# toverainc/willow-inference-server

Measured on NVIDIA H100. Metric: Whisper large-v2 realtime multiple (audio s / s), beam 5, 3.84 s utterance, higher is better.
Workload: dtype f16

## Files before the change

willow_inference_server_b200/csrc/decoder.cuh:

```cuda
#pragma once
#include "common.cuh"
#include "kernels.h"

namespace wisb {

constexpr int DEC_MAX_ROWS = 8;
constexpr int MAX_BEAM = 8;
constexpr int MAX_CAND = 2 * MAX_BEAM;
constexpr int TOPK_CHUNKS = 32;

struct DecState {
  int pos;
  int gen_step;
  int n_done;
  int all_done;
  int ticket;
};

enum GemvEpi : int {
  GV_STORE = 0,
  GV_RESID = 1,
  GV_GELU = 2,
  GV_QKV = 3,
};
// ... 16 lines not shown
  int* cand_idx = nullptr;
  int* tokens = nullptr;
  int* seq[2] = {nullptr, nullptr};
  int* indir[2] = {nullptr, nullptr};
  int* flip = nullptr;
  int* done = nullptr;
  int* n_hyp = nullptr;
  float* best_score = nullptr;
  int* best_len = nullptr;
  int* best_tokens = nullptr;
  DecState* st = nullptr;
  int* row_pos = nullptr;
  int* row_slot = nullptr;
  const int* max_new_u = nullptr;
  float rep_penalty = 1.f;
  int no_repeat_ngram = 0;
  const int* beam_u = nullptr;
  const int* max_hyp_u = nullptr;
  const float* lp_u = nullptr;
  int sample = 0;
  int topk = 0;
  float temperature = 1.f;
  const unsigned long long* seed_u = nullptr;
};
void search_step_run(const SearchArgs& a, cudaStream_t stream);
void prefill_advance_run(int* tokens, const int* prompt , int prompt_len, int R, int beam,
                         DecState* st, cudaStream_t stream);
void search_init_run(const SearchArgs& a, const int* prompt, cudaStream_t stream, int shared_prefix = 0);
void prefill_rows_run(int* tokens, int* row_pos, int* row_slot, const int* prompt, int prompt_len, int n_utt, int p0,
                      int chunk, int beam, cudaStream_t stream);

struct BatchLayer {
  GemmPlan qkv, o, cq, co, fc1, fc2;
  const float *ln1g = nullptr, *ln1b = nullptr;
  const float *ob = nullptr, *ln2g = nullptr, *ln2b = nullptr;
  const float *cob = nullptr, *ln3g = nullptr, *ln3b = nullptr;
  const float *fc2b = nullptr, *next_g = nullptr, *next_b = nullptr;
  const __half* ck = nullptr;
  const __half* cv = nullptr;
  __half* kcache = nullptr;
  __half* vcache = nullptr;
};
struct BatchArgs {
  int R = 0, d = 0, H = 0, n_utt = 0, rows_per_utt = 0, t_cap = 0, t_ind = 0, prefill = 0, with_logits = 0, pdl = 0;
  int wide = 0;
  const int* tokens = nullptr;
  const int* row_pos = nullptr;
  const int* row_slot = nullptr;
  const __half* tok_emb = nullptr;
  const float* pos_emb = nullptr;
  float* x = nullptr;
// ... 106 lines not shown
```

willow_inference_server_b200/csrc/engine.cu:

```cuda
#include <stdio.h>
#include <string.h>

#include <algorithm>
#include <cmath>
#include <functional>
#include <map>
#include <memory>
#include <mutex>
#include <string>
#include <vector>

#include "../../include/wisb200.h"
#include "decoder.cuh"
#include "kernels.h"

namespace wisb {

namespace {

thread_local std::string g_last_error;

struct TensorRef {
  const uint8_t* ptr = nullptr;
  int dtype = 0, ndim = 0;
// ... 91 lines not shown
  int mel_B = 0;
  DevBuf<__half> enc_in;
  int enc_in_B = 0;
  int enc_cap = 0;
  DevBuf<__half> h1, xn, qkv, vt, ctx, hbuf, enc_out, ckv;
  DevBuf<float> x;
  GemmPlan plan_conv2, plan_ckv;
  CUtensorMap ckv_map;
  CUtensorMap ckv_map_plain;
  std::vector<EncLayerPlans> enc_plans;
  AttnPlan attn_plan;
  int plans_B = 0, plans_vmn = -1, plans_pdl = -1;
  DevBuf<float> dx, dq, dctx, dh, logits;
  DevBuf<__half> dctx16, dh16, dxn16, dq16;
  DevBuf<float> dxstat;
  DevBuf<__half> kcache, vcache;
  DevBuf<uint8_t> mask_base, mask_cur;
  std::vector<int> mask_extra;
  DevBuf<float> row_lse, cum, cand_score, best_score, lang_probs, part_max, part_sum;
  DevBuf<unsigned long long> part;
  DevBuf<int> cand_idx, tokens, seq0, seq1, ind0, ind1, flip, done, n_hyp, best_len, best_tokens, prompt_dev, lang_ids;
  DevBuf<DecState> st;
  DevBuf<int> row_pos, row_slot, max_new_u;
  DevBuf<int> beam_u, max_hyp_u;
  DevBuf<float> lp_u;
  DevBuf<unsigned long long> seed_u;
  int search_rows = 0;
  int search_gen = 0, bd_search_gen = -1;
  int batch_rows = 320, batch_pdl = 1, decoder_batch = 1, cross_tc = 1, debug_chunk = 1;
  int bd_rows = 0, bd_tcap = 0, bd_launches_step = 0;
  DevBuf<float> bx, bq, bpart, blogits;
  DevBuf<__half> bxn, bctx, bh, bkc, bvc;
  std::vector<BatchLayer> bd_layers;
  GemmPlan bd_vocab;
  int wide_prefill = 1, prefill_rows = 1024;
  int pf_rows = 0, pf_tcap = 0;
  size_t pf_layer_cache = 0;
  const __half* pf_kc = nullptr;
  DevBuf<float> px, pq, ppart;
  DevBuf<__half> pxn, pctx, ph;
  DevBuf<int> ptok, ppos, pslot;
  std::vector<BatchLayer> pf_layers;
  DevBuf<MegaLayer> mega_layers;
  DevBuf<__half> mega_img;
  int enc_pdl = 1;
  int mega_mma = 1;
// ... 260 lines not shown
    WISB_CUDA(cudaMemcpy(h->al_items.p, items.data(), A * 4, cudaMemcpyHostToDevice));
    WISB_CUDA(cudaMemcpy(h->al_head.p, heads.data(), A * 4, cudaMemcpyHostToDevice));
  }
  h->mask_base.ensure(d.n_vocab);
  h->mask_cur.ensure(d.n_vocab);
  WISB_CUDA(cudaMemcpy(h->mask_base.p, mask.data(), mask.size(), cudaMemcpyHostToDevice));
  WISB_CUDA(cudaMemcpy(h->mask_cur.p, mask.data(), mask.size(), cudaMemcpyHostToDevice));
  const size_t R = DEC_MAX_ROWS;
  h->dx.ensure(R * d.d_model, true);
  h->dq.ensure(R * d.d_model, true);
  h->dctx.ensure(R * d.d_model, true);
  h->dh.ensure(R * 4 * d.d_model, true);
  h->dctx16.ensure(R * d.d_model, true);
  h->dh16.ensure(R * 4 * d.d_model, true);
  h->dxn16.ensure(R * d.d_model, true);
  h->dq16.ensure(R * d.d_model, true);
  h->dxstat.ensure(static_cast<size_t>(h->num_sms) * R * 2, true);
  h->logits.ensure(R * d.n_vocab_pad, true);
  const size_t cache = static_cast<size_t>(d.n_dec_layers) * R * T_MAX * d.d_model;
  h->kcache.ensure(cache, true);
  h->vcache.ensure(cache, true);
  h->flip.ensure(1, true);
  h->st.ensure(1, true);
  ensure_search(h, DEC_MAX_ROWS);
  h->mega_layers.ensure(d.n_dec_layers);
  h->mega_layers_host.ensure(d.n_dec_layers);
  h->mega_flags.ensure(mega_flags_words(), true);
  h->cross_flags.ensure(static_cast<size_t>(DEC_MAX_ROWS) * d.n_heads * 16 * 32, true);
  {
    const size_t per_layer = 2ull * (3 * d.d_model + d.d_model + 4 * d.d_model);
    h->ln_fold.ensure(per_layer * d.n_dec_layers + 2ull * d.n_vocab_pad);
    for (int i = 0; i < d.n_dec_layers; ++i) {
      const DecLayerW& w = h->dec_w[i];
      float* base = h->ln_fold.p + per_layer * i;
      mega_ln_fold(w.qkvw, w.ln1g, w.ln1b, w.qkvb, base, base + 3 * d.d_model, 3 * d.d_model, d.d_model, h->stream);
      base += 6 * d.d_model;
      mega_ln_fold(w.cqw, w.ln2g, w.ln2b, w.cqb, base, base + d.d_model, d.d_model, d.d_model, h->stream);
      base += 2 * d.d_model;
      mega_ln_fold(w.fc1w, w.ln3g, w.ln3b, w.fc1b, base, base + 4 * d.d_model, 4 * d.d_model, d.d_model, h->stream);
    }
    float* vb = h->ln_fold.p + per_layer * d.n_dec_layers;
    mega_ln_fold(h->H("dec.tok_emb"), h->F("dec.ln.g"), h->F("dec.ln.b"), nullptr, vb, vb + d.n_vocab_pad, d.n_vocab, d.d_model, h->stream);
  }
  if (mega_k_chunks(4 * d.d_model) > 1) {
    const size_t per = static_cast<size_t>(4) * d.d_model * d.d_model;
    h->fc2_chunked.ensure(per * d.n_dec_layers);
// ... 314 lines not shown
  a.prompt_len = c.prompt_len;
  a.length_penalty = c.lp;
  a.row_lse = h->row_lse.p;
  a.part_max = h->part_max.p;
  a.part_sum = h->part_sum.p;
  a.cum = h->cum.p;
  a.part = h->part.p;
  a.cand_score = h->cand_score.p;
  a.cand_idx = h->cand_idx.p;
  a.tokens = h->tokens.p;
  a.seq[0] = h->seq0.p;
  a.seq[1] = h->seq1.p;
  a.indir[0] = h->ind0.p;
  a.indir[1] = h->ind1.p;
  a.flip = h->flip.p;
  a.done = h->done.p;
  a.n_hyp = h->n_hyp.p;
  a.best_score = h->best_score.p;
  a.best_len = h->best_len.p;
  a.best_tokens = h->best_tokens.p;
  a.st = h->st.p;
  a.row_pos = h->row_pos.p;
  a.row_slot = h->row_slot.p;
  a.max_new_u = c.per_utt_max_new ? h->max_new_u.p : nullptr;
  a.rep_penalty = c.rep_penalty;
  a.no_repeat_ngram = c.no_repeat_ngram;
  if (c.mixed) {
    a.beam_u = h->beam_u.p;
    a.max_hyp_u = h->max_hyp_u.p;
    a.lp_u = h->lp_u.p;
  }
  if (c.sample) {
    a.sample = 1;
    a.topk = c.topk;
    a.temperature = c.temperature;
    a.seed_u = h->seed_u.p;
  }
  if (c.ts) {
    a.ts = 1;
    a.no_ts = dm.no_timestamps;
    a.ts_begin = dm.no_timestamps + 1;
    a.ts_max_init = std::min(a.ts_begin + c.ts_max_init, dm.n_vocab - 1);
  }
  return a;
}

// ... 36 lines not shown
      m.o.shape = m.cq.shape = m.co.shape = 1;
      m.fc1.shape = 2;
      m.fc2.shape = 3;
      m.o.next_g = w.ln2g;
      m.co.next_g = w.ln3g;
      m.fc2.next_g = i + 1 < dm.n_dec_layers ? h->dec_w[i + 1].ln1g : h->F("dec.ln.g");
      const size_t dd = d;
      const __half* img = h->mega_img.p + 14 * dd * dd * i;
      m.qkv.w = img;
      m.o.w = img + 3 * dd * dd;
      m.cq.w = img + 4 * dd * dd;
      m.co.w = img + 5 * dd * dd;
      m.fc1.w = img + 6 * dd * dd;
      m.fc2.w = img + 10 * dd * dd;
    }
    bind_cross_kv(h, m, i, c.u0, c.B_total);
    m.kcache = h->kcache.p + i * layer_cache;
    m.vcache = h->vcache.p + i * layer_cache;
  }
  WISB_CUDA(cudaMemcpyAsync(h->mega_layers.p, h->mega_layers_host.p, sizeof(MegaLayer) * dm.n_dec_layers,
                            cudaMemcpyHostToDevice, h->stream));
}

void enqueue_decoder_forward(wisb_handle* h, const DecodeCfg& c, bool with_logits, bool prefill_pass = false) {
  const Dims& dm = h->dims;
  MegaArgs a;
  a.layers = h->mega_layers.p;
  a.n_layers = dm.n_dec_layers;
  a.vocab.w = h->H("dec.tok_emb");
  a.vocab.ln_g = h->F("dec.ln.g");
  {
    const size_t per_layer = 2ull * 8 * dm.d_model;
    const float* vb = h->ln_fold.p + per_layer * dm.n_dec_layers;
    a.vocab.ln_s2 = vb;
    a.vocab.bias = vb + dm.n_vocab_pad;
  }
  a.vocab.x = h->dx.p;
  a.vocab.out = h->logits.p;
  a.vocab.ldo = dm.n_vocab_pad;
  a.vocab.N = dm.n_vocab;
  a.vocab.K = dm.d_model;
  a.vocab.epi = GV_STORE;
  if (h->mega_mma) {
    a.vocab.w = h->mega_img.p + static_cast<size_t>(14) * dm.d_model * dm.d_model * dm.n_dec_layers;
    a.tc = 1;
    a.ctx16 = h->dctx16.p;
    a.xn16 = h->dxn16.p;
    a.q16 = h->dq16.p;
    a.xstat = h->dxstat.p;
    a.vocab.x16 = h->dxn16.p;
    a.vocab.shape = 4;
  }
  a.with_logits = with_logits ? 1 : 0;
  a.R = c.n_utt * c.beam;
  a.d = dm.d_model;
  a.H = dm.n_heads;
  a.n_utt = c.n_utt;
  a.beam = c.beam;
  a.t_max = T_MAX;
  a.tokens = h->tokens.p;
  if (prefill_pass) {
    a.pf_len = c.prompt_len - 1;
    a.pf_tok_stride = c.prompt_len;
    a.pf_slot_stride = c.beam;
    a.R = c.n_utt * a.pf_len;
    a.beam = a.pf_len;
    a.tokens = h->prompt_dev.p;
  }
  a.tok_emb = h->H("dec.tok_emb");
  a.pos_emb = h->F("dec.pos");
  a.x = h->dx.p;
  a.q = h->dq.p;
  a.ctx = h->dctx.p;
  a.indir0 = h->ind0.p;
  a.indir1 = h->ind1.p;
  a.flip = h->flip.p;
  a.st = h->st.p;
  a.cross_part = h->cross_part.p;
  a.cross_flags = h->cross_flags.p;
  a.epoch_base = h->mega_flags.p;
  dec_pass_run(a, h->num_sms, h->stream);
}

void enqueue_prefill(wisb_handle* h, const DecodeCfg& c) {
  enqueue_decoder_forward(h, c, false);
// ... 72 lines not shown
        out_len[o] = len;
        for (int t = 0; t < len && t < out_stride; ++t) out_ids[o * out_stride + t] = toks[static_cast<size_t>(r) * mn + t];
        if (out_score) out_score[o] = cap > 0 ? sc[k] : 0.f;
      }
    }
    return;
  }
  int* lens = h->pin_i.p + 4;
  int* toks = lens + c.n_utt;
  const int mn = c.max_new > 0 ? c.max_new : 1;
  WISB_CUDA(cudaMemcpyAsync(lens, h->best_len.p, sizeof(int) * c.n_utt, cudaMemcpyDeviceToHost, s));
  WISB_CUDA(cudaMemcpyAsync(toks, h->best_tokens.p, sizeof(int) * c.n_utt * mn, cudaMemcpyDeviceToHost, s));
  WISB_CUDA(cudaMemcpyAsync(h->pin_f.p, h->best_score.p, sizeof(float) * c.n_utt, cudaMemcpyDeviceToHost, s));
  WISB_CUDA(cudaStreamSynchronize(s));
  for (int u = 0; u < c.n_utt; ++u) {
    const int cap = c.per_utt_max_new ? max_new_host[c.u0 + u] : c.max_new;
    const int len = cap > 0 ? lens[u] : 0;
    out_len[c.u0 + u] = len;
    for (int t = 0; t < len && t < out_stride; ++t) out_ids[static_cast<size_t>(c.u0 + u) * out_stride + t] = toks[u * mn + t];
    if (out_score) out_score[c.u0 + u] = cap > 0 ? h->pin_f.p[u] : 0.f;
  }
}

void persistent_setup(wisb_handle* h, const DecodeCfg& c, const int32_t* prompts, const int* max_new_host,
                      int shared_prefix = 0) {
  upload_prompts(h, prompts, max_new_host, c);
  search_init_run(make_search_args(h, c), h->prompt_dev.p, h->stream, shared_prefix);
  upload_mega_layers(h, c);
}

int step_loop(wisb_handle* h, int max_new, bool look_ahead, const std::function<int()>& enqueue) {
  cudaStream_t s = h->stream;
  volatile int* flag = h->pin_i.p;
  flag[0] = flag[1] = 0;
  if (look_ahead && h->ev_flag[0] == nullptr) {
    WISB_CUDA(cudaEventCreateWithFlags(&h->ev_flag[0], cudaEventDisableTiming));
    WISB_CUDA(cudaEventCreateWithFlags(&h->ev_flag[1], cudaEventDisableTiming));
  }
  int steps = 0;
  for (int gs = 0; gs < max_new; ++gs) {
    h->launches += enqueue();
    ++steps;
    WISB_CUDA(cudaMemcpyAsync(const_cast<int*>(flag) + (gs & 1), &h->st.p->all_done, sizeof(int), cudaMemcpyDeviceToHost, s));
    if (!look_ahead) {
      WISB_CUDA(cudaStreamSynchronize(s));
      if (flag[gs & 1]) break;
      continue;
    }
    WISB_CUDA(cudaEventRecord(h->ev_flag[gs & 1], s));
    if (gs >= 1) {
      WISB_CUDA(cudaEventSynchronize(h->ev_flag[(gs - 1) & 1]));
      if (flag[(gs - 1) & 1]) {
        --steps;
        break;
      }
    }
  }
  return steps;
}

int wide_prefill_run(wisb_handle* h, const DecodeCfg& c, int chunk, __half* kc, __half* vc, size_t layer_cache, int t_cap);

int decode_pass(wisb_handle* h, const DecodeCfg& c, const int32_t* prompts, const int* max_new_host, int32_t* out_ids,
                int out_stride, int32_t* out_len, float* out_score) {
  int steps = 0;
  const int pf_rows = c.n_utt * (c.prompt_len - 1);
  const bool one_pass_prefill = c.prompt_len > 1 && pf_rows <= DEC_MAX_ROWS && c.prompt_len - 1 <= MAX_BEAM;
  const bool wide = h->wide_prefill && c.prompt_len - 1 > MAX_BEAM;
  persistent_setup(h, c, prompts, max_new_host, one_pass_prefill || wide ? 1 : 0);
  if (c.max_new > 0) {
    if (one_pass_prefill) {
      enqueue_decoder_forward(h, c, false, true);
      ++steps;
    } else if (wide) {
      const int chunk = std::min(c.prompt_len - 1, std::max(1, h->prefill_rows / c.n_utt));
      steps += wide_prefill_run(h, c, chunk, h->kcache.p, h->vcache.p, static_cast<size_t>(DEC_MAX_ROWS) * T_MAX * h->dims.d_model,
                                T_MAX);
    } else {
      for (int p = 0; p + 1 < c.prompt_len; ++p) {
        enqueue_prefill(h, c);
        ++steps;
      }
    }
    if (!wide) h->launches += (c.prompt_len - 1) * 2;
    steps += step_loop(h, c.max_new, true, [&] {
      enqueue_step(h, c);
      return 1 + 2;
    });
  }
  read_results(h, c, max_new_host, out_ids, out_stride, out_len, out_score);
  return steps;
}


void plan_dec_gemm(wisb_handle* h, GemmPlan& p, const __half* a, long long lda, const __half* w, int M, int N, int K,
                   GemmEpi e, bool allow_split) {
  const int mt = M / 128;
  int bn = 256;
  while (bn > 64 && (N % bn != 0 || mt * (N / bn) < 120)) bn /= 2;
  int splits = 1;
  if (allow_split) {
    const int kb = K / 64;
    while (mt * (N / bn) * splits < 120 && splits < 8 && kb % (splits * 2) == 0 && kb / (splits * 2) >= 4) splits *= 2;
    e.mode = EPI_F32;
    e.split_stride = static_cast<long long>(M) * N;
  }
  gemm_plan(p, a, lda, w, M, N, K, e, h->num_sms, bn, 0, splits);
}

void plan_batch_layers(wisb_handle* h, std::vector<BatchLayer>& layers, int Rp, float* q, __half* xn, __half* ctx,
                       __half* hid, float* part, __half* kc, __half* vc, size_t layer_cache, int t_cap, const int* row_slot,
// ... 31 lines not shown
    GemmEpi eq;
    eq.mode = EPI_F32;
    eq.bias = w.cqb;
    eq.out = q;
    eq.ldo = d;
    plan_dec_gemm(h, b.cq, xn, d, w.cqw, Rp, d, d, eq, false);
    plan_dec_gemm(h, b.co, ctx, d, w.cow, Rp, d, d, ep, true);
    GemmEpi e1;
    e1.mode = EPI_F16_GELU;
    e1.bias = w.fc1b;
    e1.out = hid;
    e1.ldo = 4 * d;
    plan_dec_gemm(h, b.fc1, xn, d, w.fc1w, Rp, 4 * d, d, e1, false);
    plan_dec_gemm(h, b.fc2, hid, 4LL * d, w.fc2w, Rp, d, 4 * d, ep, true);
  }
}

void ensure_batch(wisb_handle* h, int rows, int t_need) {
  const Dims& dm = h->dims;
  const int d = dm.d_model, L = dm.n_dec_layers;
  int Rp = round_up(rows, 128);
  int tc = round_up(t_need, 32);
  if (tc > T_MAX) tc = T_MAX;
  ensure_search(h, rows);
  if (Rp <= h->bd_rows && tc <= h->bd_tcap && h->bd_search_gen == h->search_gen) return;
  if (Rp < h->bd_rows) Rp = h->bd_rows;
  if (tc < h->bd_tcap) tc = h->bd_tcap;
  WISB_CUDA(cudaStreamSynchronize(h->stream));
  drop_graphs(h);
  const size_t M = static_cast<size_t>(Rp);
  h->bx.ensure(M * d, true);
  h->bq.ensure(M * d, true);
  h->bxn.ensure(M * d, true);
  h->bctx.ensure(M * d, true);
  h->bh.ensure(M * 4 * d, true);
  h->bpart.ensure(8 * M * d, true);
  h->blogits.ensure(M * dm.n_vocab_pad, true);
  const size_t layer_cache = M * tc * d;
  if (layer_cache * L > h->bkc.n) {
    h->bkc.release();
    h->bvc.release();
  }
  h->bkc.ensure(layer_cache * L, true);
  h->bvc.ensure(layer_cache * L, true);
  plan_batch_layers(h, h->bd_layers, Rp, h->bq.p, h->bxn.p, h->bctx.p, h->bh.p, h->bpart.p, h->bkc.p, h->bvc.p,
                    layer_cache, tc, h->row_slot.p, h->row_pos.p);
  {
// ... 140 lines not shown
    a.xn = h->pxn.p;
    a.q = h->pq.p;
    a.ctx = h->pctx.p;
    a.part = h->ppart.p;
    a.part_stride = static_cast<long long>(h->pf_rows) * h->dims.d_model;
    if (h->ckv_is_sw) a.ckv_map = &h->ckv_map_plain;
    h->launches += 1 + batch_pass_run(a, h->pf_layers.data(), L, h->stream);
  }
  return passes;
}

void bind_batch_cross_kv(wisb_handle* h, int u0, int B_total) {
  for (int i = 0; i < h->dims.n_dec_layers; ++i) bind_cross_kv(h, h->bd_layers[i], i, u0, B_total);
}

int decode_batch(wisb_handle* h, const DecodeCfg& c, const int32_t* prompts, const int* max_new_host, int32_t* out_ids,
                 int out_stride, int32_t* out_len, float* out_score) {
  cudaStream_t s = h->stream;
  ensure_batch(h, c.n_utt * c.beam, c.prompt_len + c.max_new);
  bind_batch_cross_kv(h, c.u0, c.B_total);
  int steps = 0;
  upload_prompts(h, prompts, max_new_host, c);
  if (c.max_new > 0) {
    const int chunk_max = std::max(1, std::min(h->bd_rows / c.n_utt, MAX_BEAM));
    const int wide = std::min(c.prompt_len - 1, std::max(chunk_max, h->prefill_rows / c.n_utt));
    if (h->wide_prefill && c.prompt_len - 1 > MAX_BEAM && wide > chunk_max)
      steps += wide_prefill_run(h, c, wide, h->bkc.p, h->bvc.p, static_cast<size_t>(h->bd_rows) * h->bd_tcap * h->dims.d_model,
                                h->bd_tcap);
    else
      steps += batch_prefill(h, c, c.prompt_len, c.prompt_len - 1, chunk_max, c.beam, false);
    search_init_run(make_batch_search_args(h, c), h->prompt_dev.p, s, 1);
    cudaGraphExec_t g = nullptr;
    if (h->use_graphs && !h->profile) {
      GraphKey key;
      memset(&key, 0, sizeof(key));
      key.n_utt = c.n_utt; key.beam = c.beam; key.prompt_len = c.prompt_len; key.max_new = c.max_new;
      key.max_hyp = c.mixed ? 0 : c.max_hyp; key.lp = c.mixed ? 0.f : c.lp; key.u0 = c.u0; key.b_total = c.B_total;
      key.mixed = c.mixed;
      key.per_utt_max_new = c.per_utt_max_new;
      key.ts = c.ts; key.ts_max_init = c.ts ? c.ts_max_init : 0;
      key.rep_penalty = c.rep_penalty; key.no_repeat_ngram = c.no_repeat_ngram;
      key.sample = c.sample; key.topk = c.sample ? c.topk : 0; key.temperature = c.sample ? c.temperature : 0.f;
      auto it = h->graphs.find(key);
      if (it == h->graphs.end()) {
        if (h->graphs.size() > 64) drop_graphs(h);
        cudaGraph_t graph;
        cudaGraphExec_t exec;
        WISB_CUDA(cudaStreamBeginCapture(s, cudaStreamCaptureModeThreadLocal));
        enqueue_batch_step(h, c);
        WISB_CUDA(cudaStreamEndCapture(s, &graph));
        WISB_CUDA(cudaGraphInstantiate(&exec, graph, 0));
        WISB_CUDA(cudaGraphDestroy(graph));
        it = h->graphs.emplace(key, exec).first;
      }
      g = it->second;
    }
    steps += step_loop(h, c.max_new, false, [&] {
      if (g) WISB_CUDA(cudaGraphLaunch(g, s)); else enqueue_batch_step(h, c);
      return h->bd_launches_step;
    });
  }
  read_results(h, c, max_new_host, out_ids, out_stride, out_len, out_score);
  return steps;
}

constexpr size_t ALIGN_WS_BYTES = 2ull << 30;

void align_group(wisb_handle* h, int g0, int n, const int32_t* start_seq, int S, const int32_t* text, const int32_t* text_len,
                 int text_stride, const int32_t* num_frames, int width, int n_max, int f_max, int32_t* out_path,
                 int path_stride, int32_t* out_path_len, float* out_token_probs, float* cap_out) {
  const Dims& dm = h->dims;
  cudaStream_t s = h->stream;
  const int A = h->al_A;
  int n_grp = 0;
  for (int u = 0; u < n; ++u) n_grp = std::max(n_grp, static_cast<int>(text_len[g0 + u]));
  const int total = S + 1 + n_grp;
  int P = round_up(total, MAX_BEAM);
  if (P > dm.n_text_ctx) P = dm.n_text_ctx;
  ensure_batch(h, n * MAX_BEAM, P);
  bind_batch_cross_kv(h, 0, n);
  const int ts = std::max(text_stride, 1);
  std::vector<int> tok(static_cast<size_t>(n) * P, dm.eot), nt(n), nf(n), txt(static_cast<size_t>(n) * ts, 0);
  for (int u = 0; u < n; ++u) {
// ... 927 lines not shown
    a.row_pos = d_i.p + o_rpos;
    a.row_slot = d_slot.p;
    a.done = d_i.p + o_done;
    a.n_hyp = d_i.p + o_nhyp;
    a.best_len = d_i.p + o_blen;
    a.best_tokens = d_i.p + o_btok;
    a.cum = d_f.p;
    a.best_score = d_f.p + R;
    a.max_new_u = max_new_u ? d_cap.p : nullptr;
    a.rep_penalty = rep_penalty;
    a.no_repeat_ngram = no_repeat_ngram;
    if (mixed) {
      a.beam_u = d_beam.p;
      a.max_hyp_u = d_hyp.p;
      a.lp_u = d_lp.p;
    }
    if (sample) {
      a.sample = 1;
      a.topk = topk;
      a.temperature = temperature;
      a.seed_u = d_seed.p;
    }
    static_assert(sizeof(DecState) == 5 * sizeof(int), "DecState is five ints");
    if (init) search_init_run(a, d_prompt.p, s, init - 1);
    search_step_run(a, s);
    WISB_CUDA(cudaMemcpyAsync(state_i, d_i.p, sizeof(int) * n_i, cudaMemcpyDeviceToHost, s));
    WISB_CUDA(cudaMemcpyAsync(state_f, d_f.p, sizeof(float) * n_f, cudaMemcpyDeviceToHost, s));
    WISB_CUDA(cudaMemcpyAsync(cand_idx, d_ci.p, sizeof(int) * n_utt * MAX_CAND, cudaMemcpyDeviceToHost, s));
    WISB_CUDA(cudaMemcpyAsync(cand_score, d_cs.p, sizeof(float) * n_utt * MAX_CAND, cudaMemcpyDeviceToHost, s));
    WISB_CUDA(cudaMemcpyAsync(row_lse, d_lse.p, sizeof(float) * R, cudaMemcpyDeviceToHost, s));
    WISB_CUDA(cudaStreamSynchronize(s));
  });
}

static void align_impl(wisb_handle* h, const float* mel, int B, const int32_t* start_seq, int start_len, const int32_t* text,
                       const int32_t* text_len, int text_stride, const int32_t* num_frames, int median_filter_width,
                       int32_t* out_path, int path_stride, int32_t* out_path_len, float* out_token_probs, float* cap_out) {
    const Dims& dm = h->dims;
    WISB_REQUIRE(h->blob != nullptr, "handle has no model (created by wisb_create_frontend)");
    WISB_REQUIRE(B >= 1 && B <= 4096, "B out of range");
    WISB_REQUIRE(start_seq != nullptr && text_len != nullptr && num_frames != nullptr && out_path != nullptr &&
                 out_path_len != nullptr && out_token_probs != nullptr, "NULL argument");
    WISB_REQUIRE(start_len >= 1 && start_seq[0] == dm.sot, "start_sequence must begin with <|startoftranscript|>");
    for (int i = 0; i < start_len; ++i)
      WISB_REQUIRE(start_seq[i] >= 0 && start_seq[i] < dm.no_timestamps,
                   "start_sequence must not contain <|notimestamps|> or timestamp tokens");
    WISB_REQUIRE(median_filter_width >= 1 && median_filter_width <= 31 && median_filter_width % 2 == 1,
// ... 496 lines not shown
    DecodeCfg c;
    c.u0 = 0; c.n_utt = n_utt; c.B_total = n_utt; c.beam = beam; c.prompt_len = pf_len + 1; c.max_new = 1; c.max_hyp = 1; c.lp = 1.f;
    const DecState st{pf_len > 0 ? 0 : pos, 0, 0, 0, 0};
    WISB_CUDA(cudaMemcpyAsync(h->st.p, &st, sizeof(DecState), cudaMemcpyHostToDevice, s));
    WISB_CUDA(cudaMemcpyAsync(h->flip.p, &flip, sizeof(int), cudaMemcpyHostToDevice, s));
    std::vector<int> prompt;
    if (pf_len > 0) {
      prompt.assign(static_cast<size_t>(n_utt) * c.prompt_len, 0);
      for (int r = 0; r < R; ++r) prompt[(r / pf_len) * c.prompt_len + r % pf_len] = tokens[r];
      WISB_CUDA(cudaMemcpyAsync(h->prompt_dev.p, prompt.data(), prompt.size() * sizeof(int), cudaMemcpyHostToDevice, s));
    } else {
      WISB_CUDA(cudaMemcpyAsync(h->tokens.p, tokens, R * sizeof(int), cudaMemcpyHostToDevice, s));
      WISB_CUDA(cudaMemcpyAsync(h->ind0.p, indir0, static_cast<size_t>(R) * T_MAX * sizeof(int), cudaMemcpyHostToDevice, s));
      WISB_CUDA(cudaMemcpyAsync(h->ind1.p, indir1, static_cast<size_t>(R) * T_MAX * sizeof(int), cudaMemcpyHostToDevice, s));
    }
    const size_t cache = static_cast<size_t>(L) * DEC_MAX_ROWS * T_MAX * d;
    const size_t xs = static_cast<size_t>(DEC_MAX_ROWS) * d, ls = static_cast<size_t>(DEC_MAX_ROWS) * dm.n_vocab_pad;
    WISB_CUDA(cudaMemcpyAsync(h->kcache.p, kcache, cache * sizeof(__half), cudaMemcpyHostToDevice, s));
    WISB_CUDA(cudaMemcpyAsync(h->vcache.p, vcache, cache * sizeof(__half), cudaMemcpyHostToDevice, s));
    WISB_CUDA(cudaMemcpyAsync(h->dx.p, x, xs * sizeof(float), cudaMemcpyHostToDevice, s));
    WISB_CUDA(cudaMemcpyAsync(h->logits.p, logits, ls * sizeof(float), cudaMemcpyHostToDevice, s));
    try {
      upload_mega_layers(h, c);
      enqueue_decoder_forward(h, c, with_logits != 0, pf_len > 0);
    } catch (...) {
      h->mega_mma = saved_mma;
      throw;
    }
    h->mega_mma = saved_mma;
    WISB_CUDA(cudaMemcpyAsync(kcache, h->kcache.p, cache * sizeof(__half), cudaMemcpyDeviceToHost, s));
    WISB_CUDA(cudaMemcpyAsync(vcache, h->vcache.p, cache * sizeof(__half), cudaMemcpyDeviceToHost, s));
    WISB_CUDA(cudaMemcpyAsync(x, h->dx.p, xs * sizeof(float), cudaMemcpyDeviceToHost, s));
    WISB_CUDA(cudaMemcpyAsync(logits, h->logits.p, ls * sizeof(float), cudaMemcpyDeviceToHost, s));
    WISB_CUDA(cudaStreamSynchronize(s));
  });
}

}
```

willow_inference_server_b200/csrc/search.cu:

```cuda
#include "decoder.cuh"

namespace wisb {

namespace {

__device__ __forceinline__ unsigned f2ord(float f) {
  unsigned u = __float_as_uint(f);
  return (u & 0x80000000u) ? ~u : (u | 0x80000000u);
}
__device__ __forceinline__ float ord2f(unsigned u) {
  return __uint_as_float((u & 0x80000000u) ? (u & 0x7fffffffu) : ~u);
}
__device__ __forceinline__ unsigned long long pack_key(float score, unsigned idx) {
  return (static_cast<unsigned long long>(f2ord(score)) << 32) | static_cast<unsigned long long>(~idx);
}

__device__ __forceinline__ unsigned philox4x32_10_w0(unsigned c0, unsigned c1, unsigned c2, unsigned c3, unsigned k0,
                                                    unsigned k1) {
#pragma unroll
  for (int i = 0; i < 10; ++i) {
    const unsigned hi0 = __umulhi(0xD2511F53u, c0), lo0 = 0xD2511F53u * c0;
    const unsigned hi1 = __umulhi(0xCD9E8D57u, c2), lo1 = 0xCD9E8D57u * c2;
    c0 = hi1 ^ c1 ^ k0;
    c1 = lo1;
    c2 = hi0 ^ c3 ^ k1;
    c3 = lo0;
    k0 += 0x9E3779B9u;
    k1 += 0xBB67AE85u;
  }
  return c0;
}

__device__ __forceinline__ float gumbel_noise(unsigned long long seed, int k, int gen, int v) {
  const unsigned x = philox4x32_10_w0(static_cast<unsigned>(v), static_cast<unsigned>(gen), static_cast<unsigned>(k), 0u,
                                      static_cast<unsigned>(seed), static_cast<unsigned>(seed >> 32));
  const float u = (static_cast<float>(x >> 9) + 0.5f) * 0x1p-23f;
  return -logf(-logf(u));
}

__device__ __forceinline__ unsigned long long warp_max_u64(unsigned long long x) {
#pragma unroll
  for (int o = 16; o > 0; o >>= 1) {
    const unsigned long long y = __shfl_xor_sync(0xffffffffu, x, o);
    x = y > x ? y : x;
  }
  return x;
}

__device__ __forceinline__ float masked_logit(const SearchArgs& a, const float* row, int v, bool first_step) {
  const unsigned char m = a.mask[v];
  if ((m & 1) || (first_step && (m & 2))) return -INFINITY;
  return row[v];
}

struct TsRule {
  int lo, hi;
  int text_off;
  int below_eot_off;
  int ts_off;
};

__device__ __forceinline__ TsRule ts_rule_state(const SearchArgs& a, int r, int gen) {
  const int lane = threadIdx.x & 31;
  const int* hist = a.seq[*a.flip] + static_cast<long long>(r) * a.max_new;
  int last = -1;
  for (int t = lane; t < gen; t += 32)
    if (hist[t] >= a.ts_begin) last = t;
#pragma unroll
  for (int o = 16; o > 0; o >>= 1) last = max(last, __shfl_xor_sync(0xffffffffu, last, o));
// ... 75 lines not shown
    for (int i = tid; i <= gen - n; i += TK_THREADS) {
      bool same = true;
      for (int j = 0; j < n - 1 && same; ++j) same = s_hist[i + j] == s_hist[gen - n + 1 + j];
      const int v = s_hist[i + n - 1];
      if (same && v >= v0 && v < v1) ban[v - v0] = 1;
    }
  __syncthreads();
}

__device__ __forceinline__ float hist_logit(const SearchArgs& a, float x, unsigned char pen, unsigned char ban) {
  if (pen) x = x < 0.f ? x * a.rep_penalty : x / a.rep_penalty;
  return ban ? -INFINITY : x;
}

template <int NCH, bool HIST, bool SAMPLE = false>
__global__ void __launch_bounds__(TK_THREADS) topk_partial_kernel(const SearchArgs a) {
  constexpr bool TS = NCH > TOPK_CHUNKS;
  __shared__ unsigned long long s_red[32];
  __shared__ float s_f[32];
  __shared__ TsRule s_rule;
  if (a.st->all_done) return;
  const int chunk = blockIdx.x, r = blockIdx.y;
  const bool first = a.st->gen_step == 0;
  const float* row = a.logits + static_cast<long long>(r) * a.ldl;
  int v0, v1;
  if (!TS) {
    const int per_chunk = (a.n_vocab + TOPK_CHUNKS - 1) / TOPK_CHUNKS;
    v0 = chunk * per_chunk;
    v1 = min(a.n_vocab, v0 + per_chunk);
  } else if (chunk < TOPK_CHUNKS) {
    const int per_chunk = (a.ts_begin + TOPK_CHUNKS - 1) / TOPK_CHUNKS;
    v0 = chunk * per_chunk;
    v1 = min(a.ts_begin, v0 + per_chunk);
  } else {
    v0 = a.ts_begin;
    v1 = a.n_vocab;
  }
  const int tid = threadIdx.x, lane = tid & 31, warp = tid >> 5;
  const unsigned char* pen = nullptr;
  const unsigned char* ban = nullptr;
  if constexpr (HIST) {
    __shared__ int s_hist[HIST_MAX];
    __shared__ __align__(16) unsigned char s_pen[TK_THREADS * TK_PER];
    __shared__ __align__(16) unsigned char s_ban[TK_THREADS * TK_PER];
    hist_flags(a, r, v0, v1, s_hist, s_pen, s_ban);
    pen = s_pen;
    ban = s_ban;
// ... 151 lines not shown
    const unsigned long long key = s_out[threadIdx.x];
    const bool valid = key != 0ull && (!MIXED || static_cast<int>(threadIdx.x) < n_cand);
    a.cand_score[u * MAX_CAND + threadIdx.x] = valid ? ord2f(static_cast<unsigned>(key >> 32)) : -INFINITY;
    a.cand_idx[u * MAX_CAND + threadIdx.x] = valid ? static_cast<int>(~static_cast<unsigned>(key & 0xffffffffull)) : -1;
  }
}

template <bool MIXED>
__device__ __forceinline__ void search_bookkeeping_body(const SearchArgs& a, int* s_pick, int& s_best_k, int& s_finished) {
  const int u = blockIdx.x, lane = threadIdx.x;
  const int rows = a.beam;
  const int beam = MIXED ? a.beam_u[u] : a.beam, V = a.n_vocab, nc = MIXED ? 2 * beam : a.n_cand;
  const int gen = a.st->gen_step, pos = a.st->pos;
  const int cur = *a.flip, nxt_buf = cur ^ 1;
  const int* seq_cur = a.seq[cur];
  int* seq_nxt = a.seq[nxt_buf];
  const int* ind_cur = a.indir[cur];
  int* ind_nxt = a.indir[nxt_buf];

  if (a.done[u]) {
    for (int k = 0; k < rows; ++k) {
      const int r = u * rows + k;
      for (int t = lane; t < a.max_new; t += 32) seq_nxt[r * a.max_new + t] = seq_cur[r * a.max_new + t];
      for (int t = lane; t < a.t_max; t += 32) ind_nxt[r * a.t_max + t] = (t == pos) ? r : ind_cur[r * a.t_max + t];
    }
    return;
  }
  const float* cs = a.cand_score + u * MAX_CAND;
  const int* ci = a.cand_idx + u * MAX_CAND;
  const int cap = a.max_new_u != nullptr ? a.max_new_u[u] : a.max_new;
  const bool is_last = gen + 1 >= cap;
  const bool capped = gen >= cap;
  const float lp = MIXED ? a.lp_u[u] : a.length_penalty;
  const float norm = (lp != 0.f) ? powf(static_cast<float>(gen + 1), lp) : 1.f;
  if (lane == 0) {
    int n_hyp = a.n_hyp[u];
    float best = a.best_score[u];
    int best_k = -1;
    int secondary = beam;
    for (int k = 0; k < beam; ++k) {
      int pick = k;
      const int idx = ci[k];
      const int tok = idx < 0 ? a.eot : idx % V;
      if (!capped && idx >= 0 && (tok == a.eot || is_last)) {
        ++n_hyp;
        if (cs[k] > best) {
          best = cs[k];
// ... 25 lines not shown
    const int idx = ci[k];
    const int parent = idx / V, tok = idx % V;
    const int pr = u * rows + parent;
    for (int t = lane; t < gen; t += 32) a.best_tokens[u * a.max_new + t] = seq_cur[pr * a.max_new + t];
    if (lane == 0) {
      int len = gen;
      if (tok != a.eot) {
        a.best_tokens[u * a.max_new + gen] = tok;
        len = gen + 1;
      }
      a.best_len[u] = len;
    }
  }
  for (int k = 0; k < rows; ++k) {
    const int r = u * rows + k;
    const int idx = (!MIXED || k < beam) ? ci[s_pick[k]] : -1;
    const int parent = idx < 0 ? k : idx / V;
    const int tok = idx < 0 ? a.eot : idx % V;
    const int pr = u * rows + parent;
    for (int t = lane; t < gen; t += 32) seq_nxt[r * a.max_new + t] = seq_cur[pr * a.max_new + t];
    for (int t = lane; t < pos; t += 32) ind_nxt[r * a.t_max + t] = ind_cur[pr * a.t_max + t];
    if (lane == 0) {
      if (gen < a.max_new) seq_nxt[r * a.max_new + gen] = tok;
      ind_nxt[r * a.t_max + pos] = pr;
      a.tokens[r] = tok;
      a.cum[r] = (idx < 0) ? -INFINITY : cs[s_pick[k]] * norm;
    }
  }
}

__device__ __forceinline__ void step_advance(const SearchArgs& a, int& s_last) {
  if (threadIdx.x == 0) {
    __threadfence();
    const int t = atomicAdd(&a.st->ticket, 1);
    s_last = t == static_cast<int>(gridDim.x) - 1;
  }
  __syncthreads();
  if (s_last) {
    if (threadIdx.x == 0) {
      if (atomicAdd(&a.st->n_done, 0) == a.n_utt) a.st->all_done = 1;
      a.st->ticket = 0;
      a.st->pos += 1;
      a.st->gen_step += 1;
      *a.flip ^= 1;
    }
    if (a.row_pos != nullptr)
      for (int i = threadIdx.x; i < a.n_utt * a.beam; i += blockDim.x) a.row_pos[i] += 1;
// ... 100 lines not shown
        }
        unsigned long long pk = 0ull;
        float lm = -INFINITY;
        if (mine != 0ull) {
          lm = ord2f(static_cast<unsigned>(mine >> 32));
          const unsigned v = ~static_cast<unsigned>(mine & 0xffffffffull);
          const float key = __fdiv_rn(lm, a.temperature) + gumbel_noise(a.seed_u[u], k, gen, static_cast<int>(v));
          pk = pack_key(key, v);
        }
        best = warp_max_u64(pk);
        const unsigned owner = __ballot_sync(0xffffffffu, pk == best && best != 0ull);
        best_l = __shfl_sync(0xffffffffu, lm, owner ? __ffs(owner) - 1 : 0);
      }
    }
    const bool has = best != 0ull;
    const int tok = has ? static_cast<int>(~static_cast<unsigned>(best & 0xffffffffull)) : a.eot;
    const float cum_new = has ? (best_l - lse) + cum : -INFINITY;
    const bool finish = has && (tok == a.eot || is_last);
    if (finish)
      for (int t2 = lane; t2 < gen; t2 += 32) a.best_tokens[static_cast<long long>(r) * a.max_new + t2] = seq_cur[t2];
    if (lane == 0) {
      a.row_lse[r] = lse;
      if (gen < a.max_new) seq_nxt[gen] = tok;
      ind_nxt[pos] = r;
      if (finish) {
        int len = gen;
        if (tok != a.eot) {
          a.best_tokens[static_cast<long long>(r) * a.max_new + gen] = tok;
          len = gen + 1;
        }
        const float lp = a.length_penalty;
        const float norm = (lp != 0.f) ? powf(static_cast<float>(gen + 1), lp) : 1.f;
        a.best_len[r] = len;
        a.best_score[r] = cum_new / norm;
      }
      const bool cont = has && !finish;
      a.tokens[r] = cont ? tok : a.eot;
      a.cum[r] = cont ? cum_new : -INFINITY;
      a.cand_idx[u * MAX_CAND + k] = has ? tok : -1;
      a.cand_score[u * MAX_CAND + k] = has ? ord2f(static_cast<unsigned>(best >> 32)) : -INFINITY;
      s_live[k] = cont ? 1 : 0;
    }
  }
  __syncthreads();
  if (threadIdx.x == 0 && !frozen) {
    int any = 0;
    for (int j = 0; j < n; ++j) any |= s_live[j];
// ... 4 lines not shown
  }
  __syncthreads();
  step_advance(a, s_last);
}

__global__ void prefill_rows_kernel(int* tokens, int* row_pos, int* row_slot, const int* prompt, int prompt_len, int rows,
                                    int p0, int chunk, int beam) {
  const int i = blockIdx.x * blockDim.x + threadIdx.x;
  if (i >= rows) return;
  const int u = i / chunk, p = p0 + i % chunk;
  tokens[i] = prompt[u * prompt_len + p];
  row_pos[i] = p;
  row_slot[i] = u * beam;
}

__global__ void prefill_advance_kernel(int* tokens, const int* prompt, int prompt_len, int R, int beam, DecState* st) {
  const int next = st->pos + 1;
  for (int r = threadIdx.x; r < R; r += blockDim.x) tokens[r] = prompt[(r / beam) * prompt_len + next];
  __syncthreads();
  if (threadIdx.x == 0) st->pos = next;
}

template <bool MIXED, bool SAMPLE = false>
__global__ void search_init_kernel(const SearchArgs a, const int* prompt, int shared_prefix) {
  const int R = a.n_utt * a.beam;
  const int tid = blockIdx.x * blockDim.x + threadIdx.x, n = gridDim.x * blockDim.x;
  if (tid == 0) {
    a.st->pos = shared_prefix ? a.prompt_len - 1 : 0;
    a.st->gen_step = 0;
    a.st->n_done = 0;
    a.st->all_done = 0;
    a.st->ticket = 0;
    *a.flip = 0;
  }
  for (int i = tid; i < R; i += n) {
    const bool dead = MIXED && i % a.beam >= a.beam_u[i / a.beam];
    a.tokens[i] = dead ? a.eot : prompt[(i / a.beam) * a.prompt_len + (shared_prefix ? a.prompt_len - 1 : 0)];
    a.cum[i] = dead ? -INFINITY : 0.f;
    if (a.row_pos != nullptr) {
      a.row_pos[i] = shared_prefix ? a.prompt_len - 1 : 0;
      a.row_slot[i] = i;
    }
  }
  for (int i = tid; i < a.n_utt; i += n) {
    a.done[i] = 0;
    a.n_hyp[i] = 0;
    a.best_score[i] = -INFINITY;
    a.best_len[i] = 0;
  }
  if constexpr (SAMPLE)
    for (int i = tid; i < R; i += n) {
      a.best_score[i] = -INFINITY;
      a.best_len[i] = 0;
    }
  for (int i = tid; i < R * a.t_max; i += n) {
    const int r = i / a.t_max;
    const int slot = shared_prefix ? (r / a.beam) * a.beam : r;
    a.indir[0][i] = slot;
    a.indir[1][i] = slot;
  }
}

__global__ void lang_probs_kernel(const float* logits, long long ldl, const int* lang_ids, int n_lang, int row_stride,
                                  float* probs) {
  __shared__ float s_v[128];
  const int u = blockIdx.x;
  const float* row = logits + static_cast<long long>(u) * row_stride * ldl;
  float mx = -INFINITY;
  for (int i = threadIdx.x; i < n_lang; i += blockDim.x) {
    s_v[i] = row[lang_ids[i]];
  }
  __syncthreads();
  if (threadIdx.x == 0) {
    for (int i = 0; i < n_lang; ++i) mx = fmaxf(mx, s_v[i]);
    float s = 0.f;
    for (int i = 0; i < n_lang; ++i) s += expf(s_v[i] - mx);
    for (int i = 0; i < n_lang; ++i) probs[u * n_lang + i] = expf(s_v[i] - mx) / s;
  }
}

// ... 53 lines not shown
      topk_partial_kernel<TOPK_CHUNKS, true><<<dim3(TOPK_CHUNKS, R), TK_THREADS, 0, stream>>>(a);
    else
      topk_partial_kernel<TOPK_CHUNKS, false><<<dim3(TOPK_CHUNKS, R), TK_THREADS, 0, stream>>>(a);
    if (mixed)
      search_tail_kernel<TOPK_CHUNKS, true><<<a.n_utt, TK_THREADS, 0, stream>>>(a);
    else
      search_tail_kernel<TOPK_CHUNKS, false><<<a.n_utt, TK_THREADS, 0, stream>>>(a);
  }
  WISB_CUDA(cudaGetLastError());
}

void prefill_rows_run(int* tokens, int* row_pos, int* row_slot, const int* prompt, int prompt_len, int n_utt, int p0,
                      int chunk, int beam, cudaStream_t stream) {
  const int rows = n_utt * chunk;
  prefill_rows_kernel<<<cdiv(rows, 256), 256, 0, stream>>>(tokens, row_pos, row_slot, prompt, prompt_len, rows, p0, chunk, beam);
  WISB_CUDA(cudaGetLastError());
}

void prefill_advance_run(int* tokens, const int* prompt, int prompt_len, int R, int beam, DecState* st, cudaStream_t stream) {
  prefill_advance_kernel<<<1, 64, 0, stream>>>(tokens, prompt, prompt_len, R, beam, st);
  WISB_CUDA(cudaGetLastError());
}

void search_init_run(const SearchArgs& a, const int* prompt, cudaStream_t stream, int shared_prefix) {
  if (a.sample)
    search_init_kernel<false, true><<<8, 256, 0, stream>>>(a, prompt, shared_prefix);
  else if (a.beam_u != nullptr)
    search_init_kernel<true><<<8, 256, 0, stream>>>(a, prompt, shared_prefix);
  else
    search_init_kernel<false><<<8, 256, 0, stream>>>(a, prompt, shared_prefix);
  WISB_CUDA(cudaGetLastError());
}

void lang_probs_run(const float* logits, long long ldl, const int* lang_ids, int n_lang, int n_utt, int row_stride,
                    float* probs, cudaStream_t stream) {
  WISB_REQUIRE(n_lang <= 128, "detect_language: more than 128 language ids");
  lang_probs_kernel<<<n_utt, 128, 0, stream>>>(logits, ldl, lang_ids, n_lang, row_stride, probs);
  WISB_CUDA(cudaGetLastError());
}

}
```

Measured before the change: 131.7.

## Fuse prompt prefill with first decode step by forwarding all prompt positions

When the whole prompt fits in the row budget, the prefill pass now forwards every prompt position, including the last, and computes logits. The first search step then reads the logits of each utterance's last prompt row, so one full decoder forward per utterance is skipped. KV indirection entries for positions still inside the prompt point to the shared prefix slot. The cost is extra logic in the search kernels and a new device-side prompt_fed counter; correctness depends on the indirection and logits-row remapping being consistent.

```diff
diff --git a/willow_inference_server_b200/csrc/decoder.cuh b/willow_inference_server_b200/csrc/decoder.cuh
--- a/willow_inference_server_b200/csrc/decoder.cuh
+++ b/willow_inference_server_b200/csrc/decoder.cuh
@@ -62,11 +62,12 @@
   int topk = 0;
   float temperature = 1.f;
   const unsigned long long* seed_u = nullptr;
+  int* prompt_fed = nullptr;
 };
 void search_step_run(const SearchArgs& a, cudaStream_t stream);
 void prefill_advance_run(int* tokens, const int* prompt , int prompt_len, int R, int beam,
                          DecState* st, cudaStream_t stream);
-void search_init_run(const SearchArgs& a, const int* prompt, cudaStream_t stream, int shared_prefix = 0);
+void search_init_run(const SearchArgs& a, const int* prompt, cudaStream_t stream, int fed = 0);
 void prefill_rows_run(int* tokens, int* row_pos, int* row_slot, const int* prompt, int prompt_len, int n_utt, int p0,
                       int chunk, int beam, cudaStream_t stream);
 
diff --git a/willow_inference_server_b200/csrc/engine.cu b/willow_inference_server_b200/csrc/engine.cu
--- a/willow_inference_server_b200/csrc/engine.cu
+++ b/willow_inference_server_b200/csrc/engine.cu
@@ -137,6 +137,7 @@
   DevBuf<int> cand_idx, tokens, seq0, seq1, ind0, ind1, flip, done, n_hyp, best_len, best_tokens, prompt_dev, lang_ids;
   DevBuf<DecState> st;
   DevBuf<int> row_pos, row_slot, max_new_u;
+  DevBuf<int> prompt_fed;
   DevBuf<int> beam_u, max_hyp_u;
   DevBuf<float> lp_u;
   DevBuf<unsigned long long> seed_u;
@@ -443,6 +444,7 @@
   h->vcache.ensure(cache, true);
   h->flip.ensure(1, true);
   h->st.ensure(1, true);
+  h->prompt_fed.ensure(1, true);
   ensure_search(h, DEC_MAX_ROWS);
   h->mega_layers.ensure(d.n_dec_layers);
   h->mega_layers_host.ensure(d.n_dec_layers);
@@ -803,6 +805,7 @@
   a.st = h->st.p;
   a.row_pos = h->row_pos.p;
   a.row_slot = h->row_slot.p;
+  a.prompt_fed = h->prompt_fed.p;
   a.max_new_u = c.per_utt_max_new ? h->max_new_u.p : nullptr;
   a.rep_penalty = c.rep_penalty;
   a.no_repeat_ngram = c.no_repeat_ngram;
@@ -885,7 +888,7 @@
                             cudaMemcpyHostToDevice, h->stream));
 }
 
-void enqueue_decoder_forward(wisb_handle* h, const DecodeCfg& c, bool with_logits, bool prefill_pass = false) {
+void enqueue_decoder_forward(wisb_handle* h, const DecodeCfg& c, bool with_logits, int pf_len = 0) {
   const Dims& dm = h->dims;
   MegaArgs a;
   a.layers = h->mega_layers.p;
@@ -922,8 +925,8 @@
   a.beam = c.beam;
   a.t_max = T_MAX;
   a.tokens = h->tokens.p;
-  if (prefill_pass) {
-    a.pf_len = c.prompt_len - 1;
+  if (pf_len > 0) {
+    a.pf_len = pf_len;
     a.pf_tok_stride = c.prompt_len;
     a.pf_slot_stride = c.beam;
     a.R = c.n_utt * a.pf_len;
@@ -1042,14 +1045,13 @@
   }
 }
 
-void persistent_setup(wisb_handle* h, const DecodeCfg& c, const int32_t* prompts, const int* max_new_host,
-                      int shared_prefix = 0) {
+void persistent_setup(wisb_handle* h, const DecodeCfg& c, const int32_t* prompts, const int* max_new_host, int fed = 0) {
   upload_prompts(h, prompts, max_new_host, c);
-  search_init_run(make_search_args(h, c), h->prompt_dev.p, h->stream, shared_prefix);
+  search_init_run(make_search_args(h, c), h->prompt_dev.p, h->stream, fed);
   upload_mega_layers(h, c);
 }
 
-int step_loop(wisb_handle* h, int max_new, bool look_ahead, const std::function<int()>& enqueue) {
+int step_loop(wisb_handle* h, int max_new, bool look_ahead, const std::function<int(int gs)>& enqueue) {
   cudaStream_t s = h->stream;
   volatile int* flag = h->pin_i.p;
   flag[0] = flag[1] = 0;
@@ -1059,7 +1061,7 @@
   }
   int steps = 0;
   for (int gs = 0; gs < max_new; ++gs) {
-    h->launches += enqueue();
+    h->launches += enqueue(gs);
     ++steps;
     WISB_CUDA(cudaMemcpyAsync(const_cast<int*>(flag) + (gs & 1), &h->st.p->all_done, sizeof(int), cudaMemcpyDeviceToHost, s));
     if (!look_ahead) {
@@ -1084,29 +1086,35 @@
 int decode_pass(wisb_handle* h, const DecodeCfg& c, const int32_t* prompts, const int* max_new_host, int32_t* out_ids,
                 int out_stride, int32_t* out_len, float* out_score) {
   int steps = 0;
-  const int pf_rows = c.n_utt * (c.prompt_len - 1);
-  const bool one_pass_prefill = c.prompt_len > 1 && pf_rows <= DEC_MAX_ROWS && c.prompt_len - 1 <= MAX_BEAM;
-  const bool wide = h->wide_prefill && c.prompt_len - 1 > MAX_BEAM;
-  persistent_setup(h, c, prompts, max_new_host, one_pass_prefill || wide ? 1 : 0);
+  const int P = c.prompt_len;
+  const bool fused = c.n_utt * P <= DEC_MAX_ROWS && P <= MAX_BEAM;
+  const bool one_pass_prefill = !fused && P > 1 && c.n_utt * (P - 1) <= DEC_MAX_ROWS && P - 1 <= MAX_BEAM;
+  const bool wide = h->wide_prefill && P - 1 > MAX_BEAM;
+  persistent_setup(h, c, prompts, max_new_host, fused ? P : one_pass_prefill || wide ? P - 1 : 0);
   if (c.max_new > 0) {
-    if (one_pass_prefill) {
-      enqueue_decoder_forward(h, c, false, true);
+    if (fused || one_pass_prefill) {
+      enqueue_decoder_forward(h, c, fused, fused ? P : P - 1);
       ++steps;
+      h->launches += 1;
     } else if (wide) {
-      const int chunk = std::min(c.prompt_len - 1, std::max(1, h->prefill_rows / c.n_utt));
+      const int chunk = std::min(P - 1, std::max(1, h->prefill_rows / c.n_utt));
       steps += wide_prefill_run(h, c, chunk, h->kcache.p, h->vcache.p, static_cast<size_t>(DEC_MAX_ROWS) * T_MAX * h->dims.d_model,
                                 T_MAX);
     } else {
-      for (int p = 0; p + 1 < c.prompt_len; ++p) {
+      for (int p = 0; p + 1 < P; ++p) {
         enqueue_prefill(h, c);
         ++steps;
+        h->launches += 2;
       }
     }
-    if (!wide) h->launches += (c.prompt_len - 1) * 2;
-    steps += step_loop(h, c.max_new, true, [&] {
+    steps += step_loop(h, c.max_new, true, [&](int gs) {
+      if (fused && gs == 0) {
+        search_step_run(make_search_args(h, c), h->stream);
+        return 2;
+      }
       enqueue_step(h, c);
       return 1 + 2;
-    });
+    }) - (fused ? 1 : 0);
   }
   read_results(h, c, max_new_host, out_ids, out_stride, out_len, out_score);
   return steps;
@@ -1184,7 +1192,7 @@
   int Rp = round_up(rows, 128);
   int tc = round_up(t_need, 32);
   if (tc > T_MAX) tc = T_MAX;
-  ensure_search(h, rows);
+  ensure_search(h, std::max(Rp, h->bd_rows));
   if (Rp <= h->bd_rows && tc <= h->bd_tcap && h->bd_search_gen == h->search_gen) return;
   if (Rp < h->bd_rows) Rp = h->bd_rows;
   if (tc < h->bd_tcap) tc = h->bd_tcap;
@@ -1371,14 +1379,18 @@
   int steps = 0;
   upload_prompts(h, prompts, max_new_host, c);
   if (c.max_new > 0) {
+    const int P = c.prompt_len;
     const int chunk_max = std::max(1, std::min(h->bd_rows / c.n_utt, MAX_BEAM));
-    const int wide = std::min(c.prompt_len - 1, std::max(chunk_max, h->prefill_rows / c.n_utt));
-    if (h->wide_prefill && c.prompt_len - 1 > MAX_BEAM && wide > chunk_max)
+    const bool fused = P <= chunk_max;
+    const int wide = std::min(P - 1, std::max(chunk_max, h->prefill_rows / c.n_utt));
+    if (fused)
+      steps += batch_prefill(h, c, P, P, chunk_max, c.beam, true);
+    else if (h->wide_prefill && P - 1 > MAX_BEAM && wide > chunk_max)
       steps += wide_prefill_run(h, c, wide, h->bkc.p, h->bvc.p, static_cast<size_t>(h->bd_rows) * h->bd_tcap * h->dims.d_model,
                                 h->bd_tcap);
     else
-      steps += batch_prefill(h, c, c.prompt_len, c.prompt_len - 1, chunk_max, c.beam, false);
-    search_init_run(make_batch_search_args(h, c), h->prompt_dev.p, s, 1);
+      steps += batch_prefill(h, c, P, P - 1, chunk_max, c.beam, false);
+    search_init_run(make_batch_search_args(h, c), h->prompt_dev.p, s, fused ? P : P - 1);
     cudaGraphExec_t g = nullptr;
     if (h->use_graphs && !h->profile) {
       GraphKey key;
@@ -1404,10 +1416,14 @@
       }
       g = it->second;
     }
-    steps += step_loop(h, c.max_new, false, [&] {
+    steps += step_loop(h, c.max_new, false, [&](int gs) {
+      if (fused && gs == 0) {
+        search_step_run(make_batch_search_args(h, c), s);
+        return 2;
+      }
       if (g) WISB_CUDA(cudaGraphLaunch(g, s)); else enqueue_batch_step(h, c);
       return h->bd_launches_step;
-    });
+    }) - (fused ? 1 : 0);
   }
   read_results(h, c, max_new_host, out_ids, out_stride, out_len, out_score);
   return steps;
@@ -2381,7 +2397,7 @@
       a.seed_u = d_seed.p;
     }
     static_assert(sizeof(DecState) == 5 * sizeof(int), "DecState is five ints");
-    if (init) search_init_run(a, d_prompt.p, s, init - 1);
+    if (init) search_init_run(a, d_prompt.p, s, init == 2 ? prompt_len - 1 : 0);
     search_step_run(a, s);
     WISB_CUDA(cudaMemcpyAsync(state_i, d_i.p, sizeof(int) * n_i, cudaMemcpyDeviceToHost, s));
     WISB_CUDA(cudaMemcpyAsync(state_f, d_f.p, sizeof(float) * n_f, cudaMemcpyDeviceToHost, s));
@@ -2924,7 +2940,7 @@
     WISB_CUDA(cudaMemcpyAsync(h->logits.p, logits, ls * sizeof(float), cudaMemcpyHostToDevice, s));
     try {
       upload_mega_layers(h, c);
-      enqueue_decoder_forward(h, c, with_logits != 0, pf_len > 0);
+      enqueue_decoder_forward(h, c, with_logits != 0, pf_len);
     } catch (...) {
       h->mega_mma = saved_mma;
       throw;
diff --git a/willow_inference_server_b200/csrc/search.cu b/willow_inference_server_b200/csrc/search.cu
--- a/willow_inference_server_b200/csrc/search.cu
+++ b/willow_inference_server_b200/csrc/search.cu
@@ -45,6 +45,10 @@
     x = y > x ? y : x;
   }
   return x;
+}
+
+__device__ __forceinline__ int kv_slot(const SearchArgs& a, int pos, int prefix, int own) {
+  return a.prompt_fed != nullptr && pos < *a.prompt_fed ? prefix : own;
 }
 
 __device__ __forceinline__ float masked_logit(const SearchArgs& a, const float* row, int v, bool first_step) {
@@ -166,7 +170,10 @@
   if (a.st->all_done) return;
   const int chunk = blockIdx.x, r = blockIdx.y;
   const bool first = a.st->gen_step == 0;
-  const float* row = a.logits + static_cast<long long>(r) * a.ldl;
+  const long long lrow = first && a.prompt_fed != nullptr && *a.prompt_fed == a.prompt_len
+                             ? static_cast<long long>(r / a.beam) * a.prompt_len + a.prompt_len - 1
+                             : r;
+  const float* row = a.logits + lrow * a.ldl;
   int v0, v1;
   if (!TS) {
     const int per_chunk = (a.n_vocab + TOPK_CHUNKS - 1) / TOPK_CHUNKS;
@@ -364,7 +371,8 @@
     for (int k = 0; k < rows; ++k) {
       const int r = u * rows + k;
       for (int t = lane; t < a.max_new; t += 32) seq_nxt[r * a.max_new + t] = seq_cur[r * a.max_new + t];
-      for (int t = lane; t < a.t_max; t += 32) ind_nxt[r * a.t_max + t] = (t == pos) ? r : ind_cur[r * a.t_max + t];
+      for (int t = lane; t < a.t_max; t += 32)
+        ind_nxt[r * a.t_max + t] = (t == pos) ? kv_slot(a, pos, u * rows, r) : ind_cur[r * a.t_max + t];
     }
     return;
   }
@@ -436,7 +444,7 @@
     for (int t = lane; t < pos; t += 32) ind_nxt[r * a.t_max + t] = ind_cur[pr * a.t_max + t];
     if (lane == 0) {
       if (gen < a.max_new) seq_nxt[r * a.max_new + gen] = tok;
-      ind_nxt[r * a.t_max + pos] = pr;
+      ind_nxt[r * a.t_max + pos] = kv_slot(a, pos, u * rows, pr);
       a.tokens[r] = tok;
       a.cum[r] = (idx < 0) ? -INFINITY : cs[s_pick[k]] * norm;
     }
@@ -583,7 +591,7 @@
     if (lane == 0) {
       a.row_lse[r] = lse;
       if (gen < a.max_new) seq_nxt[gen] = tok;
-      ind_nxt[pos] = r;
+      ind_nxt[pos] = kv_slot(a, pos, u * n, r);
       if (finish) {
         int len = gen;
         if (tok != a.eot) {
@@ -634,23 +642,25 @@
 }
 
 template <bool MIXED, bool SAMPLE = false>
-__global__ void search_init_kernel(const SearchArgs a, const int* prompt, int shared_prefix) {
+__global__ void search_init_kernel(const SearchArgs a, const int* prompt, int fed) {
   const int R = a.n_utt * a.beam;
   const int tid = blockIdx.x * blockDim.x + threadIdx.x, n = gridDim.x * blockDim.x;
+  const int pos0 = min(fed, a.prompt_len - 1);
   if (tid == 0) {
-    a.st->pos = shared_prefix ? a.prompt_len - 1 : 0;
+    a.st->pos = pos0;
     a.st->gen_step = 0;
     a.st->n_done = 0;
     a.st->all_done = 0;
     a.st->ticket = 0;
     *a.flip = 0;
+    if (a.prompt_fed != nullptr) *a.prompt_fed = fed;
   }
   for (int i = tid; i < R; i += n) {
     const bool dead = MIXED && i % a.beam >= a.beam_u[i / a.beam];
-    a.tokens[i] = dead ? a.eot : prompt[(i / a.beam) * a.prompt_len + (shared_prefix ? a.prompt_len - 1 : 0)];
+    a.tokens[i] = dead ? a.eot : prompt[(i / a.beam) * a.prompt_len + pos0];
     a.cum[i] = dead ? -INFINITY : 0.f;
     if (a.row_pos != nullptr) {
-      a.row_pos[i] = shared_prefix ? a.prompt_len - 1 : 0;
+      a.row_pos[i] = pos0;
       a.row_slot[i] = i;
     }
   }
@@ -667,7 +677,7 @@
     }
   for (int i = tid; i < R * a.t_max; i += n) {
     const int r = i / a.t_max;
-    const int slot = shared_prefix ? (r / a.beam) * a.beam : r;
+    const int slot = fed > 0 ? (r / a.beam) * a.beam : r;
     a.indir[0][i] = slot;
     a.indir[1][i] = slot;
   }
@@ -767,13 +777,14 @@
   WISB_CUDA(cudaGetLastError());
 }
 
-void search_init_run(const SearchArgs& a, const int* prompt, cudaStream_t stream, int shared_prefix) {
+void search_init_run(const SearchArgs& a, const int* prompt, cudaStream_t stream, int fed) {
+  WISB_REQUIRE(fed >= 0 && fed <= a.prompt_len, "search: more prompt positions forwarded than the prompt has");
   if (a.sample)
-    search_init_kernel<false, true><<<8, 256, 0, stream>>>(a, prompt, shared_prefix);
+    search_init_kernel<false, true><<<8, 256, 0, stream>>>(a, prompt, fed);
   else if (a.beam_u != nullptr)
-    search_init_kernel<true><<<8, 256, 0, stream>>>(a, prompt, shared_prefix);
+    search_init_kernel<true><<<8, 256, 0, stream>>>(a, prompt, fed);
   else
-    search_init_kernel<false><<<8, 256, 0, stream>>>(a, prompt, shared_prefix);
+    search_init_kernel<false><<<8, 256, 0, stream>>>(a, prompt, fed);
   WISB_CUDA(cudaGetLastError());
 }
 
```

New measurement: 137.3 (median of 6 runs). 1.04x the previous value.
